# aouyang1/go-muse

Measured on NVIDIA B200. Metric: series-samples/sec (and % HBM roofline) for Batch.Run at 1/2/4/8 B200 vs host Go, higher is better.
Workload: dtype f64

## Files before the change

### go-muse_b200/csrc/muse_api.cu

```cuda
#include <cuda_runtime.h>

#include <algorithm>
#include <cmath>
#include <cstdarg>
#include <cstdio>
#include <cstdlib>
#include <cstring>
#include <atomic>
#include <mutex>
#include <thread>
#include <unordered_map>
#include <vector>

#include "../../include/muse_b200.h"
#include "muse_launch.h"
#include "muse_select.cuh"
#include "muse_synth.cuh"
#include "muse_xcorr.cuh"

using namespace muse;

static thread_local char g_err[512] = "";

static int fail(int code, const char *fmt, ...) {
    va_list ap;
    va_start(ap, fmt);
    vsnprintf(g_err, sizeof(g_err), fmt, ap);
    va_end(ap);
    return code;
}

static int cuda_fail(cudaError_t e, const char *call, const char *file, int line) {
    (void)cudaGetLastError();
    return fail(e == cudaErrorMemoryAllocation ? MUSE_ERR_OUT_OF_MEMORY : MUSE_ERR_CUDA, "%s failed: %s (%s:%d)", call,
                cudaGetErrorString(e), file, line);
}

#define CU(call)                                                                 \
    do {                                                                         \
        cudaError_t e_ = (call);                                                 \
        if (e_ != cudaSuccess) return cuda_fail(e_, #call, __FILE__, __LINE__); \
    } while (0)

extern "C" const char *muse_last_error(void) { return g_err; }
extern "C" const char *muse_version(void) { return "muse_b200 0.1 (sm_100a)"; }

#define MUSE_MAX_LABEL_KEYS 64
#define MUSE_SCRATCH_POOL 272
#define MUSE_MULTI_GROUP 256
#define MUSE_MULTI_SEPARATE 16
struct RunScratch {
    int64_t scratch_cap;
    double *d_score;
    int32_t *d_lag;
    int64_t *d_slot;
    unsigned long long *d_ckey, *d_skey;
    int32_t *d_cidx, *d_sidx;
    int32_t *d_clag, *d_slag;
    float *d_U;
    int32_t *d_list;
    float *d_L;
    signed char *d_W;
    int64_t d_L_cap;
    unsigned char *h_pin;
    size_t h_pin_bytes;
    unsigned long long *d_counters;
    SelectState *d_sel;
    int32_t *d_flag;
    unsigned *d_cut;
    int64_t table_cap;
    unsigned long long *d_gmax, *d_hkeys;
    int32_t *d_gidx;
    int64_t tab_n, d_ref_cap;
    int tab_screen;
    double *d_ref;
    cd *Xt, *twM, *twn;
    cf *twp_f;
    cf *twi_f;
    float2 *swtw;
    float4 *sw_f;
    float4 *sx_f;
    float *sb_f;
    float *d_mid;
    cudaEvent_t ev[4];
};

struct muse_ctx {
    int device;
    int sm_count;
    cudaStream_t stream;
    cudaStream_t own_stream;
    std::mutex mu;
    std::vector<RunScratch> pool;
    unsigned char *h_stage[3];
    cudaEvent_t stage_ev[3];
    double *d_roll;
    size_t d_roll_bytes;
    unsigned char *tc_a, *tc_b;
    size_t tc_a_bytes;
    float *tc_mid, *tc_amid;
    int64_t tc_mid_cap;
    void **tc_ptrs;
    unsigned *d_multi_next;
    unsigned char *d_mt, *h_mt;
    int64_t mt_top_n;
    cudaEvent_t mt_ev[5];
    int64_t multi_refined, multi_rescored;
    void *d_multi_q;
    double *d_multi_refs;
    int64_t d_multi_ld, d_multi_n;
};

struct muse_group {
    muse_ctx *ctx;
    int64_t N;
    int64_t ld;
    int64_t cap, size;
    double *slab;
    int nkeys;
    int32_t *labels;
    int32_t max_id[MUSE_MAX_LABEL_KEYS];
    int64_t global_offset;
    RowStat *row_stat;
    int64_t stats_cap, stats_upto;
};

struct muse_batch : RunScratch {
    muse_ctx *ctx;
    muse_group *g;
    int64_t N, n;
    int log2m;
    int screen_ok;
    float a_mid;
    cf x_mid;
    muse_timing timing;
    int timing_pending;
    int fused_run;
    int prescreened;
    int signed_run;
    int is_long;
    void *d_long;
    size_t d_long_bytes;
    long long long_pairs;
};

static inline cudaStream_t bstream(const muse_batch *b) { return b->ctx->stream; }

extern "C" int muse_ctx_create(int device, muse_ctx **out) {
    if (!out) return fail(MUSE_ERR_INVALID_ARG, "muse_ctx_create: out is NULL");
    int count = 0;
    cudaError_t e = cudaGetDeviceCount(&count);
    if (e != cudaSuccess || count == 0)
        return fail(MUSE_ERR_NO_DEVICE, "no CUDA device (%s); muse_b200 has no CPU fallback",
                    e != cudaSuccess ? cudaGetErrorString(e) : "device count is 0");
    if (device < 0 || device >= count) return fail(MUSE_ERR_INVALID_ARG, "device %d out of range [0,%d)", device, count);
    CU(cudaSetDevice(device));
    muse_ctx *c = new muse_ctx();
    c->device = device;
    CU(cudaDeviceGetAttribute(&c->sm_count, cudaDevAttrMultiProcessorCount, device));
    CU(cudaStreamCreateWithFlags(&c->own_stream, cudaStreamNonBlocking));
// ... 510 lines not shown
    int rc = roll_check(g, first, n_rows, samples, k, "muse_group_roll");
    if (rc != MUSE_OK || k == 0 || n_rows == 0) return rc;
    const size_t row_bytes = sizeof(double) * (size_t)k;
    if (row_bytes > MUSE_STAGE_BYTES) return fail(MUSE_ERR_UNSUPPORTED, "muse_group_roll: %lld new samples per row exceed the %zu-byte staging buffer",
                                                  (long long)k, MUSE_STAGE_BYTES);
    muse_ctx *c = g->ctx;
    CU(cudaSetDevice(c->device));
    cudaStream_t st = c->stream;
    const int64_t rows_per_chunk = stage_rows_per_chunk(k);
    const size_t want = row_bytes * (size_t)std::min<int64_t>(n_rows, rows_per_chunk);
    if (c->d_roll_bytes < want) {
        CU(cudaStreamSynchronize(st));
        cudaFree(c->d_roll);
        c->d_roll = nullptr;
        c->d_roll_bytes = 0;
        CU(cudaMalloc(&c->d_roll, want));
        c->d_roll_bytes = want;
    }
    auto queue = [&](int64_t r0, int64_t nr, const double *src) {
        cudaError_t e = cudaMemcpyAsync(c->d_roll, src, (size_t)nr * row_bytes, cudaMemcpyHostToDevice, st);
        if (e == cudaSuccess) e = launch_roll_rows(g->slab, g->ld, (int)g->N, first + r0, nr, c->d_roll, (int)k, g->row_stat, c->sm_count, st);
        return e;
    };
    cudaPointerAttributes attr;
    const bool pinned = cudaPointerGetAttributes(&attr, samples) == cudaSuccess &&
                        (attr.type == cudaMemoryTypeHost || attr.type == cudaMemoryTypeManaged);
    (void)cudaGetLastError();
    if (pinned) {
        for (int64_t r0 = 0; r0 < n_rows; r0 += rows_per_chunk)
            CU(queue(r0, std::min<int64_t>(rows_per_chunk, n_rows - r0), samples + (size_t)r0 * (size_t)k));
    } else {
        rc = stage_rows(c, samples, n_rows, k, queue);
        if (rc != MUSE_OK) return rc;
    }
    CU(cudaStreamSynchronize(st));
    return MUSE_OK;
}

static int64_t next_pow2(int64_t v) {
    int64_t n = 1;
    while (n < v) n <<= 1;
    return n;
}

static int screen_is_fused(int log2m) { return log2m >= 6 && log2m <= 13; }
static int screen_is_big(int log2m) { return log2m >= 11 && log2m <= 13; }

__global__ void screen_tables_kernel(const cd *__restrict__ Xt, int M, const float2 *__restrict__ swtw, float4 *__restrict__ sw,
                                     float4 *__restrict__ sx, float *__restrict__ sb, float *__restrict__ mid,
                                     const int32_t *__restrict__ std_zero) {
    const int k = blockIdx.x * blockDim.x + threadIdx.x;
    if (k > M / 2) return;
    if (k == 0) mid[0] = __int_as_float(*std_zero);
    const cd a = Xt[k], c = Xt[M - k];
    if (k == M / 2) {
        mid[1] = __double2float_ru(hypot(a.x, a.y) * 2.0);
        mid[2] = (float)a.x;
        mid[3] = (float)a.y;
        return;
    }
    const float wa = __double2float_ru(hypot(a.x, a.y) * (k == 0 ? 1.0 : 2.0));
    const float wc = __double2float_ru(hypot(c.x, c.y) * (k == 0 ? 1.0 : 2.0));
    const float2 w = swtw[k];
    sw[k] = make_float4(w.x, w.y, wa, wc);
    sx[k] = make_float4((float)a.x, (float)a.y, (float)c.x, (float)c.y);
    sb[k] = __double2float_ru(sqrt(2.0 * ((double)wa * (double)wa + (double)wc * (double)wc)) * (1.0 + 1e-15));
}

static int ensure_ref_tables(muse_batch *b, int64_t ld) {
    const int64_t n = b->n, M = n / 2;
    cudaStream_t st = bstream(b);
    if (b->d_ref_cap < ld) {
        cudaFree(b->d_ref);
        b->d_ref = nullptr;
        CU(cudaMalloc(&b->d_ref, sizeof(double) * (size_t)ld));
        b->d_ref_cap = ld;
    }
    if (!b->d_mid) CU(cudaMalloc(&b->d_mid, sizeof(float) * 4));
    const bool want_screen = screen_is_fused(b->log2m);
    if (b->tab_n == n && (b->tab_screen || !want_screen)) return MUSE_OK;
    if (b->is_long) {
        cudaFree(b->Xt); cudaFree(b->twM); cudaFree(b->twn); cudaFree(b->twp_f); cudaFree(b->twi_f); cudaFree(b->swtw); cudaFree(b->sw_f); cudaFree(b->sx_f); cudaFree(b->sb_f);
        b->Xt = b->twM = b->twn = nullptr;
        b->twp_f = b->twi_f = nullptr; b->swtw = nullptr; b->sw_f = b->sx_f = nullptr; b->sb_f = nullptr;
        b->tab_n = 0;
        b->tab_screen = 0;
        CU(cudaMalloc(&b->Xt, sizeof(cd) * (size_t)n));
        CU(cudaMalloc(&b->twM, sizeof(cd) * (size_t)n));
        CU(launch_long_twiddles(b->twM, b->log2m + 1, st));
        b->tab_n = n;
        return MUSE_OK;
    }
    cudaFree(b->Xt); cudaFree(b->twM); cudaFree(b->twn); cudaFree(b->twp_f); cudaFree(b->twi_f); cudaFree(b->swtw); cudaFree(b->sw_f); cudaFree(b->sx_f); cudaFree(b->sb_f);
    b->Xt = b->twM = b->twn = nullptr;
    b->twp_f = b->twi_f = nullptr; b->swtw = nullptr; b->sw_f = b->sx_f = nullptr; b->sb_f = nullptr;
    b->tab_n = 0;
    b->tab_screen = 0;
    const long double PI2 = 6.283185307179586476925286766559005768L;
    const int log2p = exact_log2p(b->log2m);
    std::vector<cd> twM((size_t)M + 16);
    fill_pass_twiddles(b->log2m, log2p, twM.data(), [&](long long num, long long den) {
        return cd{(double)cosl(-PI2 * num / den), (double)sinl(-PI2 * num / den)};
    });
    std::vector<cd> twn((size_t)(M / 2 + 1));
    for (int64_t k = 0; k <= M / 2; k++) twn[(size_t)k] = cd{(double)cosl(-PI2 * k / n), (double)sinl(-PI2 * k / n)};
    CU(cudaMalloc(&b->Xt, sizeof(cd) * (size_t)(M + 1)));
    CU(cudaMalloc(&b->twM, sizeof(cd) * twM.size()));
    CU(cudaMalloc(&b->twn, sizeof(cd) * (size_t)(M / 2 + 1)));
    CU(cudaMemcpyAsync(b->twM, twM.data(), sizeof(cd) * twM.size(), cudaMemcpyHostToDevice, st));
    CU(cudaMemcpyAsync(b->twn, twn.data(), sizeof(cd) * (size_t)(M / 2 + 1), cudaMemcpyHostToDevice, st));
    std::vector<cf> twp, twi;
    std::vector<float2> swtw;
    if (want_screen) {
        if (screen_is_big(b->log2m)) {
            twi.resize((size_t)10 * (M / 32) + 31 * (M / 1024) + 1024 + 31 * 32);
            fill_big_twiddles(b->log2m, twi.data(), [&](long long num, long long den) {
                return cf{(float)cosl(-PI2 * num / den), (float)sinl(-PI2 * num / den)};
            });
            CU(cudaMalloc(&b->twi_f, sizeof(cf) * twi.size()));
            CU(cudaMemcpyAsync(b->twi_f, twi.data(), sizeof(cf) * twi.size(), cudaMemcpyHostToDevice, st));
        }
        twp.resize((size_t)M + 64);
        fill_pass_twiddles(b->log2m, 5, twp.data(), [&](long long num, long long den) {
            return cf{(float)cosl(-PI2 * num / den), (float)sinl(-PI2 * num / den)};
        });
        swtw.resize((size_t)M / 2);
        for (int64_t k = 0; k < M / 2; k++) swtw[(size_t)k] = make_float2((float)cosl(-PI2 * k / n), (float)sinl(-PI2 * k / n));
        CU(cudaMalloc(&b->twp_f, sizeof(cf) * twp.size()));
        CU(cudaMalloc(&b->swtw, sizeof(float2) * swtw.size()));
        CU(cudaMalloc(&b->sw_f, sizeof(float4) * (size_t)(M / 2)));
        CU(cudaMalloc(&b->sx_f, sizeof(float4) * (size_t)(M / 2)));
        CU(cudaMalloc(&b->sb_f, sizeof(float) * (size_t)(M / 2)));
        CU(cudaMemcpyAsync(b->twp_f, twp.data(), sizeof(cf) * twp.size(), cudaMemcpyHostToDevice, st));
        CU(cudaMemcpyAsync(b->swtw, swtw.data(), sizeof(float2) * swtw.size(), cudaMemcpyHostToDevice, st));
    }
    CU(cudaStreamSynchronize(st));
    b->tab_n = n;
    b->tab_screen = want_screen ? 1 : 0;
    return MUSE_OK;
}

extern "C" void muse_batch_destroy(muse_batch *b);
static int ensure_long_work(muse_batch *b, int64_t count);
static LongParams long_params(const muse_batch *b, const double *slab, int64_t count, const int32_t *idx, int signed_scores);

#define CUB(call)                                                          \
    do {                                                                   \
        cudaError_t e_ = (call);                                           \
        if (e_ != cudaSuccess) {                                           \
            const int rc_ = cuda_fail(e_, #call, __FILE__, __LINE__);      \
            muse_batch_destroy(b);                                         \
            return rc_;                                                    \
        }                                                                  \
    } while (0)

static int batch_alloc(muse_ctx *ctx, muse_group *g, int64_t ref_len, muse_batch **out) {
    if (!ctx || !g || !out) return fail(MUSE_ERR_INVALID_ARG, "muse_batch_create: NULL argument");
    if (g->ctx != ctx) return fail(MUSE_ERR_INVALID_ARG, "group belongs to another context");
    if (ref_len != g->N)
        return fail(MUSE_ERR_LENGTH_MISMATCH, "comparison group series (length %lld) does not have the same length as the reference (%lld)",
                    (long long)g->N, (long long)ref_len);
    const int64_t n = next_pow2(ref_len);
    if (n > MUSE_MAX_FFT_LEN) return fail(MUSE_ERR_UNSUPPORTED, "FFT length %lld > %d", (long long)n, MUSE_MAX_FFT_LEN);
    CU(cudaSetDevice(ctx->device));
    muse_batch *b = new muse_batch();
    memset(b, 0, sizeof(*b));
    b->is_long = n > MUSE_MAX_FUSED_FFT_LEN;
    b->ctx = ctx;
    b->g = g;
    b->N = ref_len;
    b->n = n;
    const int64_t M = n / 2;
    int l = 0;
    while ((1LL << l) < M) l++;
    b->log2m = l;
    {
        std::lock_guard<std::mutex> lk(ctx->mu);
        if (!ctx->pool.empty()) {
            size_t best = 0;
            auto better = [&](const RunScratch &x, const RunScratch &y) {
                if ((x.tab_n == n) != (y.tab_n == n)) return x.tab_n == n;
                return x.scratch_cap > y.scratch_cap;
            };
            for (size_t i = 1; i < ctx->pool.size(); i++)
                if (better(ctx->pool[i], ctx->pool[best])) best = i;
            static_cast<RunScratch &>(*b) = ctx->pool[best];
            ctx->pool.erase(ctx->pool.begin() + (long)best);
        }
    }
    auto bail = [&](int code) {
        muse_batch_destroy(b);
        return code;
    };
    for (int i = 0; i < 4; i++)
        if (!b->ev[i] && cudaEventCreate(&b->ev[i]) != cudaSuccess) return bail(fail(MUSE_ERR_CUDA, "cudaEventCreate failed"));
    int rc = ensure_ref_tables(b, g->ld);
    if (rc) return bail(rc);
    cudaError_t e = cudaSuccess;
    if (!b->d_flag) e = cudaMalloc(&b->d_flag, sizeof(int32_t));
    if (e == cudaSuccess && !b->d_counters) e = cudaMalloc(&b->d_counters, sizeof(unsigned long long) * 4);
    if (e == cudaSuccess && !b->d_sel) e = cudaMalloc(&b->d_sel, sizeof(SelectState));
    if (e == cudaSuccess && !b->d_cut) e = cudaMalloc(&b->d_cut, sizeof(unsigned) * (4 + MUSE_CUT_WORDS));
    if (e == cudaSuccess && !b->h_pin) {
        b->h_pin_bytes = (size_t)4 << 20;
        e = cudaHostAlloc((void **)&b->h_pin, b->h_pin_bytes, cudaHostAllocDefault);
    }
    if (e != cudaSuccess) {
        (void)cudaGetLastError();
        return bail(fail(e == cudaErrorMemoryAllocation ? MUSE_ERR_OUT_OF_MEMORY : MUSE_ERR_CUDA, "muse_batch_create: %s", cudaGetErrorString(e)));
    }
    *out = b;
    return MUSE_OK;
}

static int batch_create_queue(muse_ctx *ctx, muse_group *g, const double *ref, int64_t ref_len, muse_batch **out,
                              const double *d_ref_row = nullptr) {
// ... 1819 lines not shown
```

### go-muse_b200/csrc/muse_screen.cuh

```cuda
#pragma once

#include <vector_functions.h>
#include <vector_types.h>

#include "muse_score.cuh"

namespace muse {

typedef cx<float> cf;

#ifndef MUSE_SCREEN_SLACK
#define MUSE_SCREEN_SLACK 1e-4f
#endif
#define MUSE_SCREEN_VAR_MIN 1e-20f
#define MUSE_SCREEN_VAR_MAX 1e28f
#define MUSE_SCREEN_OFFSET_MAX 1e8
#define MUSE_CUT_BINS 262144
#define MUSE_CUT_WORDS (64 + 64 * 64 + MUSE_CUT_BINS)

struct alignas(16) RowStat {
    double mean;
    float rstd;
    unsigned pad;
};

struct ScreenParams {
    const double *slab;
    int64_t ld;
    int64_t count;
    int N;
    const cf *twp;
    const float4 *sw;
    const float *sb;
    float a_mid;
    const float4 *sx;
    cf x_mid;
    float *out_L;
    const RowStat *row_stat;
    unsigned *cut_bits;
    unsigned *cut_hist;
    unsigned long long *n_refined;
    unsigned *next_claim;
    int top_n;
    int win_lo, win_len;
    float thr;
    int grouped;
    float *out_U;
    const cf *twi;
    const int64_t *slot_of;
    unsigned long long *group_L;
    signed char *out_W;
};

MUSE_HD bool window_row_hit(int off, int row_len, int win_lo, int win_len, int n) {
    const int d = (off - win_lo) & (n - 1);
    return d <= win_len || d > n - row_len;
}
MUSE_HD void window_pair(cx<float> r, int idx, int win_len, int nmask, bool hit, float &m_in, float &m_out) {
    const float a0 = fabsf(r.y), a1 = fabsf(r.x);
    if (hit) {
        const bool in0 = (idx & nmask) <= win_len;
        const bool in1 = ((idx + 1) & nmask) <= win_len;
        m_in = fmaxf(m_in, fmaxf(in0 ? a0 : 0.f, in1 ? a1 : 0.f));
        m_out = fmaxf(m_out, fmaxf(in0 ? 0.f : a0, in1 ? 0.f : a1));
    } else {
        m_out = fmaxf(m_out, fmaxf(a0, a1));
    }
}

#if defined(__CUDACC__)

template <int T>
__device__ __forceinline__ float group_sum_f(float x) {
#pragma unroll
    for (int off = T / 2; off > 0; off >>= 1) x += __shfl_xor_sync(0xffffffffu, x, off);
    return x;
}

__device__ __forceinline__ unsigned smem_u32(const void *p) { return (unsigned)__cvta_generic_to_shared(p); }

__device__ __forceinline__ void mbar_init(unsigned bar, unsigned count) {
    asm volatile("mbarrier.init.shared::cta.b64 [%0], %1;" ::"r"(bar), "r"(count) : "memory");
}
__device__ __forceinline__ void mbar_init_fence() { asm volatile("fence.mbarrier_init.release.cluster;" ::: "memory"); }
__device__ __forceinline__ void mbar_expect(unsigned bar, unsigned bytes) {
    asm volatile("mbarrier.arrive.expect_tx.shared::cta.b64 _, [%0], %1;" ::"r"(bar), "r"(bytes) : "memory");
}
__device__ __forceinline__ void bulk_copy(unsigned dst, const void *src, unsigned bytes, unsigned bar) {
    asm volatile("cp.async.bulk.shared::cluster.global.mbarrier::complete_tx::bytes [%0], [%1], %2, [%3];" ::"r"(dst), "l"(src),
                 "r"(bytes), "r"(bar)
                 : "memory");
}
__device__ __forceinline__ void bulk_load(unsigned dst, const void *src, unsigned bytes, unsigned bar) {
    mbar_expect(bar, bytes);
    bulk_copy(dst, src, bytes, bar);
}
__device__ __forceinline__ void mbar_wait(unsigned bar, unsigned parity) {
    unsigned done;
    do {
        asm volatile(
            "{\n"
            ".reg .pred p;\n"
            "mbarrier.try_wait.parity.shared::cta.b64 p, [%1], %2;\n"
            "selp.u32 %0, 1, 0, p;\n"
            "}\n"
            : "=r"(done)
            : "r"(bar), "r"(parity)
            : "memory");
    } while (!done);
}

__device__ __forceinline__ float sqrt_approx(float x) {
    float r;
    asm("sqrt.approx.ftz.f32 %0, %1;" : "=f"(r) : "f"(x));
    return r;
}

__device__ __forceinline__ unsigned ld_relaxed_u32(const unsigned *p) {
    unsigned r;
    asm volatile("ld.relaxed.gpu.global.u32 %0, [%1];" : "=r"(r) : "l"(p) : "memory");
    return r;
}

__device__ __forceinline__ void mbar_test(unsigned bar, unsigned parity) {
    asm volatile(
        "{\n"
        ".reg .pred p;\n"
        "mbarrier.test_wait.parity.shared::cta.b64 p, [%0], %1;\n"
        "}\n" ::"r"(bar),
        "r"(parity)
        : "memory");
}

__device__ __forceinline__ int cut_level(const unsigned *cnt, int t, unsigned &need) {
    const unsigned h = ld_relaxed_u32(&cnt[63 - 2 * t]), l = ld_relaxed_u32(&cnt[62 - 2 * t]);
    unsigned incl = h + l;
#pragma unroll
    for (int off = 1; off < 32; off <<= 1) {
        const unsigned o = __shfl_up_sync(0xffffffffu, incl, off);
        if (t >= off) incl += o;
    }
    const unsigned excl = incl - (h + l);
    const unsigned hit = __ballot_sync(0xffffffffu, incl >= need);
    if (!hit) return -1;
    const int leader = __ffs(hit) - 1;
    const bool upper = excl + h >= need;
    const int idx = upper ? 63 - 2 * t : 62 - 2 * t;
    const unsigned above = upper ? excl : excl + h;
    need -= __shfl_sync(0xffffffffu, above, leader);
    return __shfl_sync(0xffffffffu, idx, leader);
}

__device__ __forceinline__ void cut_count_and_raise(unsigned *const &cut_bits, unsigned *const &cut_hist, const int &top_n, float L, int t) {
    int bin = (int)(L * (float)MUSE_CUT_BINS);
    bin = bin < 0 ? 0 : (bin >= MUSE_CUT_BINS ? MUSE_CUT_BINS - 1 : bin);
    unsigned *coarse = cut_hist, *mid = coarse + 64, *fine = mid + 64 * 64;
    if (t == 0) {
        atomicAdd(&fine[bin], 1u);
        atomicAdd(&mid[bin >> 6], 1u);
        atomicAdd(&coarse[bin >> 12], 1u);
    }
    __syncwarp();
    unsigned need = (unsigned)top_n;
    const int c = cut_level(coarse, t, need);
    if (c < 0) return;
    const int m = cut_level(mid + c * 64, t, need);
    if (m < 0) return;
    const int f = cut_level(fine + (c * 64 + m) * 64, t, need);
    if (f < 0) return;
    if (t == 0) atomicMax(cut_bits, __float_as_uint((float)((c * 64 + m) * 64 + f) / (float)MUSE_CUT_BINS));
}

__device__ __forceinline__ float refine_decide(float U, float s_in, float s_out, float &L, int grouped) {
    if (!(s_in == s_in) || !(s_out == s_out)) return U;
    const float u32 = fminf(fmaxf(s_in, s_out) * 1.00001f, 1.f) + MUSE_SCREEN_SLACK;
    if (grouped) {
        L = fmaxf(fminf(fmaxf(s_in, s_out) * 0.99999f, 1.f) - MUSE_SCREEN_SLACK, 0.f);
        return fminf(U, u32);
    }
    if (s_out * 0.99999f - MUSE_SCREEN_SLACK > s_in * 1.00001f + MUSE_SCREEN_SLACK) return -1.f;
    if (s_in * 0.99999f - MUSE_SCREEN_SLACK > s_out * 1.00001f + MUSE_SCREEN_SLACK)
        L = fminf(s_in * 0.99999f, 1.f) - MUSE_SCREEN_SLACK;
    return fminf(U, u32);
}


template <int T>
MUSE_HD constexpr int screen_reg(int m) {
    return (m % (32 / T)) * T + Perm<T>::at(m / (32 / T));
}

template <int NZ, int T>
__device__ __forceinline__ void load_centred(cf (&v)[32], const cd *rowc, int t, double mu, bool last_in) {
#pragma unroll
    for (int r = 0; r < 32; r++) {
        if (r < NZ) {
            const cd x = (r == NZ - 1 && !last_in) ? cd{mu, mu} : rowc[t + r * T];
            v[r] = cf{(float)(x.x - mu), (float)(x.y - mu)};
        } else {
            v[r] = cf{0.f, 0.f};
        }
    }
}

template <int T>
__device__ __forceinline__ void screen_pass0(cf (&v)[32], cf *ex, const cf *const &tw, int t) {
    constexpr int LOG2M = 5 + (T >= 2) + (T >= 4) + (T >= 8) + (T >= 16) + (T >= 32);
    using G = Geo<LOG2M, 5>;
#pragma unroll
    for (int j = 0; j < 32; j++) {
        cf val = v[Perm<32>::at(j)];
        if (j > 0) val = cmul(val, tw[(j - 1) * T + t]);
        ex[G::pad(32 * t + j)] = val;
    }
    __syncwarp();
    fft_pass_load<LOG2M, 5, 1, float>(v, ex, t);
}

template <int T>
__device__ __forceinline__ void screen_pass1(cf *v) {
#pragma unroll
    for (int c = 0; c < 32 / T; c++) Dft<T, float>::run(v + c * T);
}

template <int T>
__device__ __forceinline__ cf mirror_of(const cf (&v)[32], int m, bool lane0, int partner) {
    const cf zp = v[screen_reg<T>(31 - m)];
    const cf zs = v[screen_reg<T>((32 - m) & 31)];
    cf src, zm;
    src.x = lane0 ? zs.x : zp.x;
    src.y = lane0 ? zs.y : zp.y;
    zm.x = __shfl_sync(0xffffffffu, src.x, partner, T);
    zm.y = __shfl_sync(0xffffffffu, src.y, partner, T);
    return zm;
}

__device__ __forceinline__ void split_sq(cf e, cf d, cf w, cf &qk, cf &qm) {
    const cf wo = cmul(cmul_negi(d), w);
    const cf y1 = cadd(e, wo);
    const cf y2 = csub(e, wo);
    qk = pmul(y1, y1);
    qm = pmul(y2, y2);
}

template <int T, bool PAIR>
__device__ __forceinline__ float screen_bound(const cf (&v)[32], const ScreenParams &prm, int t, bool lane0, int partner) {
    float acc = 0.f;
#pragma unroll
    for (int m = 0; m < 16; m++) {
        const cf zk = v[screen_reg<T>(m)];
        const cf zm = mirror_of<T>(v, m, lane0, partner);
        const cf zmc = cconj(zm);
        const cf e = cadd(zk, zmc);
        if constexpr (PAIR) {
            const cf d = csub(zk, zmc);
            const cf q = pfma(d, d, pmul(e, e));
            acc = fmaf(sqrt_approx(q.x + q.y), prm.sb[t + T * m], acc);
        } else {
            const float4 sv = prm.sw[t + T * m];
            cf qk, qm;
            split_sq(e, csub(zk, zmc), cf{sv.x, sv.y}, qk, qm);
            acc = fmaf(sqrt_approx(qk.x + qk.y), sv.z, fmaf(sqrt_approx(qm.x + qm.y), sv.w, acc));
        }
    }
    {
        const cf z = v[screen_reg<T>(16)];
        const cf q = pmul(z, z);
        acc = fmaf(sqrt_approx(q.x + q.y), lane0 ? 2.f * prm.a_mid : 0.f, acc);
    }
    return group_sum_f<T>(acc);
}

__device__ __forceinline__ cf split_twiddle(float4 s) { return cf{s.x, s.y}; }
__device__ __forceinline__ cf split_twiddle(cf s) { return s; }

template <int T, typename SW>
__device__ __forceinline__ void conj_mul_pairs(cf (&v)[32], const SW *const &sw, const float4 *const &sx, const cf &x_mid, int t, bool lane0,
                                               int partner) {
#pragma unroll
    for (int m = 0; m < 16; m++) {
        const cf zk = v[screen_reg<T>(m)];
        const cf zm = mirror_of<T>(v, m, lane0, partner);
        const cf w = split_twiddle(sw[t + T * m]);
        const float4 x = sx[t + T * m];
        cf ok, om;
        pointwise_pair(zk, zm, w, cf{x.x, x.y}, cf{x.z, x.w}, ok, om);
        cf rcv;
        rcv.x = __shfl_sync(0xffffffffu, om.x, partner, T);
        rcv.y = __shfl_sync(0xffffffffu, om.y, partner, T);
        v[screen_reg<T>(m)] = ok;
        cf &hi = v[screen_reg<T>(31 - m)];
        hi.x = lane0 ? hi.x : rcv.x;
        hi.y = lane0 ? hi.y : rcv.y;
        if (m > 0) {
            cf &own = v[screen_reg<T>(32 - m)];
            own.x = lane0 ? om.x : own.x;
// ... 47 lines not shown
    return r;
}

struct RowSums {
    double s1 = 0.0, s2 = 0.0;
    __device__ __forceinline__ void add(double v, double pivot) {
        const double x = v - pivot;
        s1 += x;
        s2 = fma(x, x, s2);
    }
    __device__ __forceinline__ RowStat warp_stat(double pivot, int N) {
#pragma unroll
        for (int off = 16; off > 0; off >>= 1) {
            s1 += __shfl_xor_sync(0xffffffffu, s1, off);
            s2 += __shfl_xor_sync(0xffffffffu, s2, off);
        }
        return make_row_stat(pivot, s1, s2, N);
    }
};
#endif

static __global__ void row_stats_kernel(double *__restrict__ slab, int64_t ld, int N, int64_t first, int64_t count,
                                 RowStat *__restrict__ stat) {
    const int lane = threadIdx.x & 31;
    const int64_t warp0 = ((int64_t)blockIdx.x * blockDim.x + threadIdx.x) >> 5;
    const int64_t nwarp = ((int64_t)gridDim.x * blockDim.x) >> 5;
    for (int64_t i = warp0; i < count; i += nwarp) {
        const double *row = slab + (first + i) * ld;
        const double pivot = row[0];
        RowSums rs;
        for (int k = lane; k < N; k += 32) rs.add(row[k], pivot);
        const RowStat r = rs.warp_stat(pivot, N);
        if (lane == 0) {
            stat[first + i] = r;
            if (N & 1) slab[(first + i) * ld + N] = r.mean;
        }
    }
}

struct ScreenWarpCfg {
    using G = Geo<10, 5>;
    static constexpr int MAX_WARPS = 12;
    static constexpr int NREF = 2;
    static constexpr int CLAIM = 2;
    static constexpr size_t SMEM_BUDGET = 227 * 1024;
    static constexpr size_t EX_BYTES = ((size_t)(G::MP + 1) * sizeof(cf) + 127) / 128 * 128;
    static size_t row_bytes(int N) { const size_t r = ((size_t)N * 8 + 127) / 128 * 128; return r > EX_BYTES ? r : EX_BYTES; }
    static size_t warp_bytes(int N) { return row_bytes(N); }
    static int warps(int N) {
        const size_t w = (SMEM_BUDGET - NREF * EX_BYTES) / warp_bytes(N);
        return (int)(w > MAX_WARPS ? MAX_WARPS : w);
    }
    static size_t smem_bytes(int N) { return (size_t)warps(N) * warp_bytes(N) + NREF * EX_BYTES; }
    static int nz(int N) { return ((N + 1) / 2 + 31) / 32; }
};

__device__ __forceinline__ int ex_acquire(unsigned *locks, int t, int hint) {
    int slot = hint & (ScreenWarpCfg::NREF - 1);
    while (true) {
        unsigned old = 1u;
        if (t == 0) old = atomicCAS(&locks[slot], 0u, 1u);
        if (__shfl_sync(0xffffffffu, old, 0) == 0u) break;
        slot = (slot + 1) & (ScreenWarpCfg::NREF - 1);
    }
    return slot;
}
__device__ __forceinline__ void ex_release(unsigned *locks, int t, int slot) {
    __syncwarp();
    if (t == 0) {
        __threadfence_block();
        atomicExch(&locks[slot], 0u);
    }
}

template <int NZ>
__global__ void __launch_bounds__(ScreenWarpCfg::MAX_WARPS * 32, 1)
score_screen_warp_kernel(const ScreenParams prm, const unsigned warp_bytes, const unsigned row_bytes) {
    using C = ScreenWarpCfg;
    constexpr int P = 32;
    extern __shared__ __align__(128) unsigned char smem_raw[];
    __shared__ __align__(8) unsigned long long bars[C::MAX_WARPS];
    __shared__ unsigned ex_locks[C::NREF];
    __shared__ int next_of[C::MAX_WARPS];

    const int w = threadIdx.x >> 5;
    const int t = threadIdx.x & 31;
    const int count = (int)prm.count;
    const int grid_warps = (int)(gridDim.x * (blockDim.x >> 5));
    const int pos0 = ((int)(blockIdx.x * (blockDim.x >> 5)) + w) * C::CLAIM;
    unsigned char *buf = smem_raw + (size_t)w * warp_bytes;
    const cd *rowc = reinterpret_cast<const cd *>(buf);
    cf *sm = reinterpret_cast<cf *>(buf);
    unsigned char *refbase = smem_raw + (size_t)(blockDim.x >> 5) * warp_bytes;
    const int N = prm.N;
    const int Nh = (N + 1) >> 1;
    const unsigned bar = smem_u32(&bars[w]);
    const int partner = (P - t) & (P - 1);
    const bool lane0 = (t == 0);
    const bool last_in = t + (NZ - 1) * 32 < Nh;

    if (threadIdx.x < C::NREF) ex_locks[threadIdx.x] = 0u;
    if (t == 0) {
        mbar_init(bar, 1);
        mbar_init_fence();
        if (pos0 < count) bulk_load(smem_u32(buf), prm.slab + (int64_t)pos0 * prm.ld, (unsigned)(N + (N & 1)) * 8u, bar);
    }
    __syncthreads();

    unsigned pp = (unsigned)pos0;
    while ((int)(pp & 0x7fffffffu) < count) {
        const int pos = (int)(pp & 0x7fffffffu);
        const unsigned phase = pp >> 31;
        const bool claim_ends = (pos & (C::CLAIM - 1)) == C::CLAIM - 1;
        unsigned cut_raw = 0u, claim = 0u;
        if (t == 0) {
            cut_raw = ld_relaxed_u32(prm.cut_bits);
            if (claim_ends) claim = atomicInc(prm.next_claim, (unsigned)count);
        }
        const RowStat rs = prm.row_stat[pos];
        const double mu = rs.mean;
        mbar_wait(bar, phase);

        cf v[P];
        load_centred<NZ, 32>(v, rowc, t, mu, last_in);
        __syncwarp();

        Dft32Lead<NZ, float>::run(v);
        screen_pass0<32>(v, sm, prm.twp, t);
        __syncwarp();
        if (t == 0) {
            const int next = claim_ends ? (grid_warps + (int)claim) * C::CLAIM : pos + 1;
            next_of[w] = next;
            if (next < count) {
                asm volatile("" ::"r"(__float_as_uint(v[P - 1].y)) : "memory");
                asm volatile("fence.proxy.async.shared::cta;" ::: "memory");
                bulk_load(smem_u32(buf), prm.slab + (int64_t)next * prm.ld, (unsigned)(N + (N & 1)) * 8u, bar);
            }
        }
        screen_pass1<32>(v);
        const float acc = screen_bound<32, true>(v, prm, t, lane0, partner);

        float U = acc * rs.rstd * 1.00001f + MUSE_SCREEN_SLACK;
        if (!(U == U)) U = 2.f;
        float L = -1.f;
        const int bsrc = (__float_as_uint(acc) == 0x7fc12345u) ? 1 : 0;
        const float cut_now = __uint_as_float(__shfl_sync(0xffffffffu, cut_raw, bsrc));
        if (U >= cut_now && U < 1.5f) {
#pragma unroll
            for (int j = 0; j < P / 2; j++) {
                const cf zk = v[Perm<P>::at(j)];
                const cf zm = mirror_of<32>(v, j, lane0, partner);
                const float4 s = prm.sw[t + 32 * j];
                const float4 x = prm.sx[t + 32 * j];
                cf ok, om;
                pointwise_pair(zk, zm, cf{s.x, s.y}, cf{x.x, x.y}, cf{x.z, x.w}, ok, om);
                cf rcv;
                rcv.x = __shfl_sync(0xffffffffu, om.x, partner);
                rcv.y = __shfl_sync(0xffffffffu, om.y, partner);
                v[Perm<P>::at(j)] = ok;
                cf &hi = v[Perm<P>::at(P - 1 - j)];
                hi.x = lane0 ? hi.x : rcv.x;
                hi.y = lane0 ? hi.y : rcv.y;
                if (j > 0) {
                    cf &own = v[Perm<P>::at(P - j)];
                    own.x = lane0 ? om.x : own.x;
                    own.y = lane0 ? om.y : own.y;
                }
            }
            {
                cf &mid = v[Perm<P>::at(P / 2)];
                cf ok, om;
                pointwise_pair(mid, mid, cf{0.f, -1.f}, prm.x_mid, prm.x_mid, ok, om);
                mid.x = lane0 ? ok.x : mid.x;
                mid.y = lane0 ? ok.y : mid.y;
            }
            cf u[P];
#pragma unroll
            for (int j = 0; j < P; j++) u[j] = v[Perm<P>::at(j)];
            Dft<P, float>::run(u);
            {
                const int slot = ex_acquire(ex_locks, t, w);
                screen_pass0<32>(u, reinterpret_cast<cf *>(refbase + (size_t)slot * C::EX_BYTES), prm.twp, t);
                ex_release(ex_locks, t, slot);
            }
            screen_pass1<32>(u);
            float m_in, m_out;
            window_maxima<32>(u, t, prm.win_lo, prm.win_len, m_in, m_out);
            const float rstd = rs.rstd;
            const float s_in = m_in * rstd, s_out = m_out * rstd;
            U = refine_decide(U, s_in, s_out, L, prm.grouped);
            if (t == 0) atomicAdd(prm.n_refined, 1ull);
            if (L >= prm.thr && L >= cut_now) cut_count_and_raise(prm.cut_bits, prm.cut_hist, prm.top_n, L, t);
        }
        if (t == 0) {
            prm.out_U[pos] = U;
            if (prm.out_L) prm.out_L[pos] = L;
        }
        __syncwarp();
        pp = (unsigned)next_of[w] | (~pp & 0x80000000u);
    }
}

#endif

}
```

### go-muse_b200/csrc/muse_screen_big.cuh

```cuda
#pragma once

#include "muse_screen.cuh"

namespace muse {

template <int LOG2M>
struct ScreenBigCfg {
    static_assert(LOG2M >= 11 && LOG2M <= 13, "big kernel: n = 4096, 8192, 16384");
    static constexpr int M = 1 << LOG2M;
    static constexpr int P = 32;
    static constexpr int T = M / P;
    static constexpr int NWARP = T / 32;
    static constexpr int LR = LOG2M - 10;
    static constexpr int R = 1 << LR;
    static constexpr int NB = P / R;
    static constexpr int NPAIR = NB / 2;
    static constexpr int TP = T + (T >> 5);
    static constexpr int JP = 1024 + 32;
    static constexpr int TR = T + (T >> LR);
    static constexpr int SM_ELEMS = M + (M >> LR) + 2;
    static constexpr size_t EX_BYTES = ((size_t)SM_ELEMS * 8 + 127) / 128 * 128;
#ifndef MUSE_BIG_SMEM_TW
#define MUSE_BIG_SMEM_TW 1
#endif
// ... 200 lines not shown
            }
        } else {
#pragma unroll
            for (int j = 0; j < R; j++) {
                cf &a = lo[Perm<R>::at(j)], &b = hi[Perm<R>::at(R - 1 - j)];
                cf ok, om;
                if (j < R / 2) {
                    const float4 s = big_load_f4(sw + u + 1024 * j), x = big_load_f4(sx + u + 1024 * j);
                    pointwise_pair(a, b, cf{s.x, s.y}, cf{x.x, x.y}, cf{x.z, x.w}, ok, om);
                    a = ok;
                    b = om;
                } else {
                    const int kk = M - u - 1024 * j;
                    const float4 s = big_load_f4(sw + kk), x = big_load_f4(sx + kk);
                    pointwise_pair(b, a, cf{s.x, s.y}, cf{x.x, x.y}, cf{x.z, x.w}, ok, om);
                    b = ok;
                    a = om;
                }
            }
        }
    }
}

template <int LOG2M>
MUSE_HD void big_inv_pass0(cf *v, cf *sm, int t, const cf *twi) {
    using C = ScreenBigCfg<LOG2M>;
    constexpr int R = C::R;
#pragma unroll
    for (int c2 = 0; c2 < C::NPAIR; c2++) {
        const int u = t + C::T * c2;
#pragma unroll
        for (int h = 0; h < 2; h++) {
            const int b = h == 0 ? u : big_b_hi(u);
            cf *x = v + (2 * c2 + h) * R;
            cf w[R];
#pragma unroll
            for (int j = 0; j < R; j++) w[j] = x[Perm<R>::at(j)];
            Dft<R, float>::run(w);
            cf *dst = sm + (R + 1) * b;
            dst[0] = w[Perm<R>::at(0)];
            cf pw[R];
            pw[1] = twi[C::TWI0_OFF + b];
#pragma unroll
            for (int j = 2; j < R; j++) pw[j] = cmul(pw[j / 2], pw[j - j / 2]);
#pragma unroll
            for (int j = 1; j < R; j++) dst[j] = cmul(w[Perm<R>::at(j)], pw[j]);
        }
    }
}
template <int LOG2M>
MUSE_HD void big_inv_pass1_load(cf *v, const cf *sm, int t) {
    using C = ScreenBigCfg<LOG2M>;
    const int ptr = t + (t >> C::LR);
#pragma unroll
    for (int j = 0; j < 32; j++) v[j] = sm[ptr + C::TR * j];
}
template <int LOG2M>
MUSE_HD void big_inv_pass1(cf *v, cf *sm, int t, const cf *twi) {
    using C = ScreenBigCfg<LOG2M>;
    constexpr int R = C::R;
    Dft<32, float>::run(v);
    const int p = t >> C::LR, q = t & (R - 1);
    cf *dst = sm + q + 33 * R * p;
    const cf *tw = twi + C::TWI1_OFF + p;
    dst[0] = v[Perm<32>::at(0)];
#pragma unroll
    for (int j = 1; j < 32; j++) dst[R * j + ((R * j) >> 5)] = cmul(v[Perm<32>::at(j)], tw[(j - 1) * 32]);
}
template <int LOG2M>
MUSE_HD void big_window_max(const cf *v, int t, int win_lo, int win_len, float &m_in, float &m_out) {
    using C = ScreenBigCfg<LOG2M>;
    m_in = 0.f;
    m_out = 0.f;
    const int base = 2 * t - win_lo;
#pragma unroll
    for (int j = 0; j < 32; j++) {
        const int off = 2 * C::T * j;
        window_pair(v[Perm<32>::at(j)], base + off, win_len, 2 * C::M - 1, window_row_hit(off, 2 * C::T, win_lo, win_len, 2 * C::M), m_in,
                    m_out);
    }
}

#if defined(__CUDACC__)

__device__ __forceinline__ void big_l2_prefetch(const void *p, unsigned bytes) {
    asm volatile("cp.async.bulk.prefetch.L2.global [%0], %1;" ::"l"(p), "r"(bytes) : "memory");
}

#ifndef MUSE_BIG_LOAD_BATCH
#define MUSE_BIG_LOAD_BATCH 16
#endif

template <int LOG2M, int MINB, int NZ = 0>
__global__ void __launch_bounds__(ScreenBigCfg<LOG2M>::T, MINB)
score_screen_big_kernel(const ScreenParams prm) {
    using C = ScreenBigCfg<LOG2M>;
    constexpr int P = 32, T = C::T, NW = C::NWARP, LB = MUSE_BIG_LOAD_BATCH;
    extern __shared__ __align__(128) unsigned char smem_raw[];
    __shared__ float2 red_f[2][NW];
    __shared__ unsigned bc_word[2];
    cf *sm = reinterpret_cast<cf *>(smem_raw);
#if MUSE_BIG_SMEM_TW
    cf *s_tw = reinterpret_cast<cf *>(smem_raw + C::EX_BYTES);
    for (int i = threadIdx.x; i < C::TW_SMEM; i += C::T) s_tw[i] = prm.twi[i];
    float *s_sb = reinterpret_cast<float *>(s_tw + C::TW_SMEM);
    if (C::SB_SMEM)
        for (int i = threadIdx.x; i < C::M / 2; i += C::T) s_sb[i] = prm.sb[i];
    __syncthreads();
    const cf *twf = s_tw;
    const cf *twinv = MUSE_BIG_SMEM_TW == 3 ? s_tw : prm.twi;
    const float *sbp = C::SB_SMEM ? s_sb : prm.sb;
#else
    const cf *twf = prm.twi;
    const cf *twinv = prm.twi;
    const float *sbp = prm.sb;
#endif

    const int t = threadIdx.x;
    const int N = prm.N;
    const int Nh = (N + 1) >> 1;
    const int count = (int)prm.count;
    const unsigned row_bytes = (unsigned)(N + (N & 1)) * 8u;
    const int chunk = (count + (int)gridDim.x - 1) / (int)gridDim.x;
    const int pos_lo = (int)blockIdx.x * chunk;
    const int pos_hi = min(pos_lo + chunk, count);
    if (t == 0 && pos_lo < pos_hi) big_l2_prefetch(prm.slab + (int64_t)pos_lo * prm.ld, row_bytes);

    for (int pos = pos_lo; pos < pos_hi; pos++) {
        const double *rowp = prm.slab + (int64_t)pos * prm.ld;
        unsigned cut_raw = 0u, lg_raw = 0u;
        unsigned long long *gslot = nullptr;
        if (t == 0) {
            if (pos + 1 < pos_hi) big_l2_prefetch(rowp + prm.ld, row_bytes);
            cut_raw = ld_relaxed_u32(prm.cut_bits);
            if (prm.group_L) {
                gslot = prm.group_L + prm.slot_of[pos];
                lg_raw = ld_relaxed_u32(reinterpret_cast<const unsigned *>(gslot));
            }
        }
        const RowStat rs = prm.row_stat[pos];
        const double mu = rs.mean;

        cf v[P];
#pragma unroll
        for (int b0 = 0; b0 < P; b0 += LB) {
            cd x[LB];
#pragma unroll
            for (int q = 0; q < LB; q++) {
                const int j = t + (b0 + q) * T;
if constexpr (NZ > 0) {
                    if (b0 + q < NZ - 1) x[q] = load_pair_stream(rowp + 2 * j);
                    else if (b0 + q == NZ - 1) x[q] = j < Nh ? load_pair_stream(rowp + 2 * j) : cd{mu, mu};
                    else x[q] = cd{mu, mu};
                } else {
                    x[q] = (b0 + q < P / 2 || j < Nh) ? load_pair_stream(rowp + 2 * j) : cd{mu, mu};
                }
            }
#pragma unroll
            for (int q = 0; q < LB; q++) {
                if (NZ > 0 && b0 + q >= NZ) v[b0 + q] = cf{0.f, 0.f};
                else v[b0 + q] = cf{(float)(x[q].x - mu), (float)(x[q].y - mu)};
            }
        }

        big_fwd_pass0<LOG2M, NZ == 0 ? 32 : NZ>(v, sm, t, twf);
        __syncthreads();
        big_load_stride_t<LOG2M>(v, sm, t);
        __syncthreads();
        big_fwd_pass1<LOG2M>(v, sm, t, twf);
        __syncthreads();
        big_fwd_last<LOG2M>(v, sm, t);

#if defined(MUSE_BIG_BINS)
        float acc = big_split_bound<LOG2M, false>(v, t, prm.sw, prm.a_mid, sbp);
#else
        float acc = big_split_bound<LOG2M, true>(v, t, prm.sw, prm.a_mid, sbp);
#endif
#pragma unroll
        for (int off = 16; off > 0; off >>= 1) acc += __shfl_xor_sync(0xffffffffu, acc, off);
        if ((t & 31) == 0) red_f[0][t >> 5].x = acc;
        if (t == 0) {
            bc_word[0] = cut_raw;
            bc_word[1] = lg_raw;
        }
        __syncthreads();
        acc = red_f[0][0].x;
#pragma unroll
        for (int w = 1; w < NW; w++) acc += red_f[0][w].x;
        const float cut_now = __uint_as_float(bc_word[0]);
        const float lg_now = __uint_as_float(bc_word[1]);
        float U = acc * rs.rstd * 1.00001f + MUSE_SCREEN_SLACK;
        if (!(U == U)) U = 2.f;
        float L = -1.f;
        signed char W = 0;
        if (U >= cut_now && U >= lg_now && U < 1.5f) {
            big_pointwise<LOG2M>(v, t, prm.sw, prm.sx, prm.x_mid);
            big_inv_pass0<LOG2M>(v, sm, t, twinv);
            __syncthreads();
            big_inv_pass1_load<LOG2M>(v, sm, t);
            __syncthreads();
            big_inv_pass1<LOG2M>(v, sm, t, twinv);
            __syncthreads();
            big_load_stride_t<LOG2M>(v, sm, t);
            Dft<32, float>::run(v);
            float m_in, m_out;
            big_window_max<LOG2M>(v, t, prm.win_lo, prm.win_len, m_in, m_out);
#pragma unroll
            for (int off = 16; off > 0; off >>= 1) {
                m_in = fmaxf(m_in, __shfl_xor_sync(0xffffffffu, m_in, off));
                m_out = fmaxf(m_out, __shfl_xor_sync(0xffffffffu, m_out, off));
            }
            if ((t & 31) == 0) red_f[1][t >> 5] = make_float2(m_in, m_out);
            __syncthreads();
            float2 mx = red_f[1][0];
#pragma unroll
            for (int w = 1; w < NW; w++) {
// ... 29 lines not shown
```

### go-muse_b200/csrc/muse_screen_multi.cuh

```cuda
#pragma once

#include "muse_screen.cuh"

namespace muse {

struct MultiQuery {
    const float4 *sw;
    const float4 *sx;
    cf x_mid;
    float a_mid;
    int pad;
    unsigned *cut;
    float *out_U;
};

#if defined(__CUDACC__)

struct RefineMultiCfg {
    using G = Geo<10, 5>;
#ifndef MUSE_REFINE_WARPS
#define MUSE_REFINE_WARPS 8
#endif
    static constexpr int MAX_WARPS = MUSE_REFINE_WARPS;
    static constexpr int QMAX = 256;
    static constexpr int QI = QMAX / 32;
    static constexpr size_t SMEM_BUDGET = 227 * 1024;
    static constexpr size_t STASH_BYTES = (size_t)G::M * sizeof(cf);
    static constexpr size_t EX_BYTES = ScreenWarpCfg::EX_BYTES;
    static size_t warp_bytes(int N) {
        const size_t row = ((size_t)N * 8 + 127) / 128 * 128, own = STASH_BYTES + EX_BYTES;
        return row > own ? row : own;
    }
    static constexpr size_t TW_BYTES = 31 * 32 * sizeof(cf) + 64, SW_BYTES = (size_t)(G::M / 2) * sizeof(cf);
    static size_t table_bytes() { return (size_t)QMAX * 2 * sizeof(void *) + TW_BYTES + SW_BYTES; }
    static int warps(int N) {
        const size_t w = (SMEM_BUDGET - table_bytes()) / warp_bytes(N);
        return (int)(w > MAX_WARPS ? MAX_WARPS : w);
    }
    static size_t smem_bytes(int N) { return (size_t)warps(N) * warp_bytes(N) + table_bytes(); }
};

template <int NZ>
__global__ void __launch_bounds__(RefineMultiCfg::MAX_WARPS * 32, 1)
refine_multi_kernel(const ScreenParams prm, const MultiQuery *__restrict__ queries, const int nq, const unsigned warp_bytes,
                    unsigned *__restrict__ next_series) {
    using C = RefineMultiCfg;
    constexpr int P = 32, M = C::G::M, QI = C::QI;
    extern __shared__ __align__(128) unsigned char smem_raw[];
    __shared__ __align__(8) unsigned long long bars[C::MAX_WARPS];

    const int w = threadIdx.x >> 5;
    const int t = threadIdx.x & 31;
    const int nwarps = (int)(blockDim.x >> 5);
    const int count = (int)prm.count;
    const int pos0 = (int)(blockIdx.x * nwarps) + w;
    unsigned char *buf = smem_raw + (size_t)w * warp_bytes;
    const cd *rowc = reinterpret_cast<const cd *>(buf);
    cf *stash = reinterpret_cast<cf *>(buf);
    cf *ex = reinterpret_cast<cf *>(buf + C::STASH_BYTES);
    unsigned **s_cut = reinterpret_cast<unsigned **>(smem_raw + (size_t)nwarps * warp_bytes);
    float **s_out = reinterpret_cast<float **>(s_cut + C::QMAX);
    cf *s_tw = reinterpret_cast<cf *>(s_out + C::QMAX);
    cf *s_sw = reinterpret_cast<cf *>(reinterpret_cast<unsigned char *>(s_tw) + C::TW_BYTES);
    const int N = prm.N;
    const int Nh = (N + 1) >> 1;
    const unsigned bar = smem_u32(&bars[w]);
    const int partner = (P - t) & (P - 1);
    const bool lane0 = (t == 0);
    const bool last_in = t + (NZ - 1) * 32 < Nh;
    const int nqi = (nq + 31) >> 5;

    if (t == 0) {
        mbar_init(bar, 1);
        mbar_init_fence();
        if (pos0 < count) bulk_load(smem_u32(buf), prm.slab + (int64_t)pos0 * prm.ld, (unsigned)(N + (N & 1)) * 8u, bar);
    }
    for (int q = threadIdx.x; q < C::QMAX; q += blockDim.x) {
        s_cut[q] = q < nq ? queries[q].cut : nullptr;
        s_out[q] = q < nq ? queries[q].out_U : nullptr;
    }
    for (int i = threadIdx.x; i < 31 * 32; i += blockDim.x) s_tw[i] = prm.twp[i];
    for (int i = threadIdx.x; i < M / 2; i += blockDim.x) {
        const float4 s = prm.sw[i];
        s_sw[i] = cf{s.x, s.y};
    }
    __syncthreads();

    unsigned phase = 0;
    int next = 0;
    for (int pos = pos0; pos < count; pos = next, phase ^= 1u) {
        float U[QI];
        unsigned cutr[QI];
#pragma unroll
        for (int i = 0; i < QI; i++) {
            U[i] = -1.f;
            cutr[i] = 0x7f800000u;
            if (i < nqi && t + 32 * i < nq) {
                U[i] = s_out[t + 32 * i][pos];
                cutr[i] = ld_relaxed_u32(s_cut[t + 32 * i]);
            }
        }
        const RowStat rs = prm.row_stat[pos];
        const double mu = rs.mean;
        mbar_wait(bar, phase);

        cf v[P];
        load_centred<NZ, 32>(v, rowc, t, mu, last_in);
        __syncwarp();
        if (t == 0) next = (int)atomicAdd(next_series, 1u);
        next = __shfl_sync(0xffffffffu, next, 0);

        Dft32Lead<NZ, float>::run(v);
        screen_pass0<32>(v, ex, s_tw, t);
        screen_pass1<32>(v);
#pragma unroll
        for (int j = 0; j < P; j++) stash[32 * j + t] = v[Perm<P>::at(j)];

        unsigned todo[QI];
#pragma unroll
        for (int i = 0; i < QI; i++) todo[i] = __ballot_sync(0xffffffffu, U[i] >= __uint_as_float(cutr[i]) && U[i] < 1.5f);
        unsigned changed = 0u;
#pragma unroll 1
        while (true) {
            int gi = -1;
            unsigned gm = 0u;
#pragma unroll
            for (int i = QI - 1; i >= 0; i--)
                if (todo[i]) {
                    gi = i;
                    gm = todo[i];
                }
            if (gi < 0) break;
            const int ql = __ffs(gm) - 1;
            float Usel = 0.f;
            unsigned csel = 0u;
#pragma unroll
            for (int i = 0; i < QI; i++) {
                if (i == gi) {
                    todo[i] = gm & (gm - 1);
                    Usel = U[i];
                    csel = cutr[i];
                }
            }
            {
                float Uq = __shfl_sync(0xffffffffu, Usel, ql);
                const float cut_now = __uint_as_float(__shfl_sync(0xffffffffu, csel, ql));
                const MultiQuery mq = queries[32 * gi + ql];
                cf z[P];
#pragma unroll
                for (int j = 0; j < P; j++) z[Perm<P>::at(j)] = stash[32 * j + t];
                conj_mul_pairs<32>(z, s_sw, mq.sx, mq.x_mid, t, lane0, partner);
                cf u[P];
#pragma unroll
                for (int j = 0; j < P; j++) u[j] = z[Perm<P>::at(j)];
                Dft<P, float>::run(u);
                __syncwarp();
                screen_pass0<32>(u, ex, s_tw, t);
                screen_pass1<32>(u);
                float m_in, m_out;
                window_maxima<32>(u, t, prm.win_lo, prm.win_len, m_in, m_out);
                float L = -1.f;
                Uq = refine_decide(Uq, m_in * rs.rstd, m_out * rs.rstd, L, 0);
                if (t == 0) atomicAdd(reinterpret_cast<unsigned long long *>(mq.cut + 2), 1ull);
                if (L >= prm.thr && L >= cut_now) cut_count_and_raise(mq.cut, mq.cut + 4, prm.top_n, L, t);
// ... 23 lines not shown
```

Baseline: 664.1 billion.

## Pack screen pass twiddles as float4 pairs and prefetch next claimed rows into L2

Repacks the float screen FFT pass-0 twiddle table so each thread loads two twiddles per float4 (odd/even j pairs). This halves the number of twiddle loads in screen_pass0. The single-query screen kernel now claims its next row block at the start of a claim instead of the end, and uses that early claim to issue a bulk L2 prefetch of the upcoming rows. The cost is an extra shared-memory slot per warp and an earlier atomic. The L2 prefetch helper is also shared with the big-screen kernel.

```diff
diff --git a/go-muse_b200/csrc/muse_api.cu b/go-muse_b200/csrc/muse_api.cu
--- a/go-muse_b200/csrc/muse_api.cu
+++ b/go-muse_b200/csrc/muse_api.cu
@@ -75,7 +75,7 @@
     int tab_screen;
     double *d_ref;
     cd *Xt, *twM, *twn;
-    cf *twp_f;
+    float4 *twp_f;
     cf *twi_f;
     float2 *swtw;
     float4 *sw_f;
@@ -752,7 +752,7 @@
     if (b->is_long) {
         cudaFree(b->Xt); cudaFree(b->twM); cudaFree(b->twn); cudaFree(b->twp_f); cudaFree(b->twi_f); cudaFree(b->swtw); cudaFree(b->sw_f); cudaFree(b->sx_f); cudaFree(b->sb_f);
         b->Xt = b->twM = b->twn = nullptr;
-        b->twp_f = b->twi_f = nullptr; b->swtw = nullptr; b->sw_f = b->sx_f = nullptr; b->sb_f = nullptr;
+        b->twp_f = nullptr; b->twi_f = nullptr; b->swtw = nullptr; b->sw_f = b->sx_f = nullptr; b->sb_f = nullptr;
         b->tab_n = 0;
         b->tab_screen = 0;
         CU(cudaMalloc(&b->Xt, sizeof(cd) * (size_t)n));
@@ -763,7 +763,7 @@
     }
     cudaFree(b->Xt); cudaFree(b->twM); cudaFree(b->twn); cudaFree(b->twp_f); cudaFree(b->twi_f); cudaFree(b->swtw); cudaFree(b->sw_f); cudaFree(b->sx_f); cudaFree(b->sb_f);
     b->Xt = b->twM = b->twn = nullptr;
-    b->twp_f = b->twi_f = nullptr; b->swtw = nullptr; b->sw_f = b->sx_f = nullptr; b->sb_f = nullptr;
+    b->twp_f = nullptr; b->twi_f = nullptr; b->swtw = nullptr; b->sw_f = b->sx_f = nullptr; b->sb_f = nullptr;
     b->tab_n = 0;
     b->tab_screen = 0;
     const long double PI2 = 6.283185307179586476925286766559005768L;
@@ -779,7 +779,8 @@
     CU(cudaMalloc(&b->twn, sizeof(cd) * (size_t)(M / 2 + 1)));
     CU(cudaMemcpyAsync(b->twM, twM.data(), sizeof(cd) * twM.size(), cudaMemcpyHostToDevice, st));
     CU(cudaMemcpyAsync(b->twn, twn.data(), sizeof(cd) * (size_t)(M / 2 + 1), cudaMemcpyHostToDevice, st));
-    std::vector<cf> twp, twi;
+    std::vector<float4> twp;
+    std::vector<cf> twi;
     std::vector<float2> swtw;
     if (want_screen) {
         if (screen_is_big(b->log2m)) {
@@ -790,18 +791,22 @@
             CU(cudaMalloc(&b->twi_f, sizeof(cf) * twi.size()));
             CU(cudaMemcpyAsync(b->twi_f, twi.data(), sizeof(cf) * twi.size(), cudaMemcpyHostToDevice, st));
         }
-        twp.resize((size_t)M + 64);
-        fill_pass_twiddles(b->log2m, 5, twp.data(), [&](long long num, long long den) {
-            return cf{(float)cosl(-PI2 * num / den), (float)sinl(-PI2 * num / den)};
-        });
+        const int64_t T = M / 32;
+        twp.resize((size_t)(16 * T));
+        for (int64_t i = 0; i < 16; i++)
+            for (int64_t t = 0; t < T; t++) {
+                const int64_t k1 = (2 * i + 1) * t, k2 = (2 * i + 2) * t;
+                twp[(size_t)(i * T + t)] = make_float4((float)cosl(-PI2 * k1 / M), (float)sinl(-PI2 * k1 / M), (float)cosl(-PI2 * k2 / M),
+                                                       (float)sinl(-PI2 * k2 / M));
+            }
         swtw.resize((size_t)M / 2);
         for (int64_t k = 0; k < M / 2; k++) swtw[(size_t)k] = make_float2((float)cosl(-PI2 * k / n), (float)sinl(-PI2 * k / n));
-        CU(cudaMalloc(&b->twp_f, sizeof(cf) * twp.size()));
+        CU(cudaMalloc(&b->twp_f, sizeof(float4) * twp.size()));
         CU(cudaMalloc(&b->swtw, sizeof(float2) * swtw.size()));
         CU(cudaMalloc(&b->sw_f, sizeof(float4) * (size_t)(M / 2)));
         CU(cudaMalloc(&b->sx_f, sizeof(float4) * (size_t)(M / 2)));
         CU(cudaMalloc(&b->sb_f, sizeof(float) * (size_t)(M / 2)));
-        CU(cudaMemcpyAsync(b->twp_f, twp.data(), sizeof(cf) * twp.size(), cudaMemcpyHostToDevice, st));
+        CU(cudaMemcpyAsync(b->twp_f, twp.data(), sizeof(float4) * twp.size(), cudaMemcpyHostToDevice, st));
         CU(cudaMemcpyAsync(b->swtw, swtw.data(), sizeof(float2) * swtw.size(), cudaMemcpyHostToDevice, st));
     }
     CU(cudaStreamSynchronize(st));
diff --git a/go-muse_b200/csrc/muse_screen.cuh b/go-muse_b200/csrc/muse_screen.cuh
--- a/go-muse_b200/csrc/muse_screen.cuh
+++ b/go-muse_b200/csrc/muse_screen.cuh
@@ -29,7 +29,7 @@
     int64_t ld;
     int64_t count;
     int N;
-    const cf *twp;
+    const float4 *twp;
     const float4 *sw;
     const float *sb;
     float a_mid;
@@ -91,6 +91,9 @@
                  "r"(bytes), "r"(bar)
                  : "memory");
 }
+__device__ __forceinline__ void l2_prefetch(const void *p, unsigned bytes) {
+    asm volatile("cp.async.bulk.prefetch.L2.global [%0], %1;" ::"l"(p), "r"(bytes) : "memory");
+}
 __device__ __forceinline__ void bulk_load(unsigned dst, const void *src, unsigned bytes, unsigned bar) {
     mbar_expect(bar, bytes);
     bulk_copy(dst, src, bytes, bar);
@@ -204,14 +207,16 @@
 }
 
 template <int T>
-__device__ __forceinline__ void screen_pass0(cf (&v)[32], cf *ex, const cf *const &tw, int t) {
+__device__ __forceinline__ void screen_pass0(cf (&v)[32], cf *ex, const float4 *const &tw, int t) {
     constexpr int LOG2M = 5 + (T >= 2) + (T >= 4) + (T >= 8) + (T >= 16) + (T >= 32);
     using G = Geo<LOG2M, 5>;
-#pragma unroll
-    for (int j = 0; j < 32; j++) {
-        cf val = v[Perm<32>::at(j)];
-        if (j > 0) val = cmul(val, tw[(j - 1) * T + t]);
-        ex[G::pad(32 * t + j)] = val;
+    const float4 *twt = tw + t;
+    ex[G::pad(32 * t)] = v[0];
+#pragma unroll
+    for (int j = 1; j < 32; j += 2) {
+        const float4 w = twt[(j >> 1) * T];
+        ex[G::pad(32 * t + j)] = cmul(v[Perm<32>::at(j)], cf{w.x, w.y});
+        if (j < 31) ex[G::pad(32 * t + j + 1)] = cmul(v[Perm<32>::at(j + 1)], cf{w.z, w.w});
     }
     __syncwarp();
     fft_pass_load<LOG2M, 5, 1, float>(v, ex, t);
@@ -425,6 +430,7 @@
     __shared__ __align__(8) unsigned long long bars[C::MAX_WARPS];
     __shared__ unsigned ex_locks[C::NREF];
     __shared__ int next_of[C::MAX_WARPS];
+    __shared__ int claim_of[C::MAX_WARPS];
 
     const int w = threadIdx.x >> 5;
     const int t = threadIdx.x & 31;
@@ -454,11 +460,20 @@
     while ((int)(pp & 0x7fffffffu) < count) {
         const int pos = (int)(pp & 0x7fffffffu);
         const unsigned phase = pp >> 31;
+        const bool claim_starts = (pos & (C::CLAIM - 1)) == 0;
         const bool claim_ends = (pos & (C::CLAIM - 1)) == C::CLAIM - 1;
         unsigned cut_raw = 0u, claim = 0u;
         if (t == 0) {
             cut_raw = ld_relaxed_u32(prm.cut_bits);
-            if (claim_ends) claim = atomicInc(prm.next_claim, (unsigned)count);
+            if (claim_starts) {
+                claim = atomicInc(prm.next_claim, (unsigned)count);
+            } else if (claim_ends) {
+                const int nc = claim_of[w];
+                if (nc < count) {
+                    const int rows = count - nc < C::CLAIM ? count - nc : C::CLAIM;
+                    l2_prefetch(prm.slab + (int64_t)nc * prm.ld, (unsigned)((int64_t)(rows - 1) * prm.ld + N + (N & 1)) * 8u);
+                }
+            }
         }
         const RowStat rs = prm.row_stat[pos];
         const double mu = rs.mean;
@@ -472,7 +487,8 @@
         screen_pass0<32>(v, sm, prm.twp, t);
         __syncwarp();
         if (t == 0) {
-            const int next = claim_ends ? (grid_warps + (int)claim) * C::CLAIM : pos + 1;
+            if (claim_starts) claim_of[w] = (grid_warps + (int)claim) * C::CLAIM;
+            const int next = claim_ends ? claim_of[w] : pos + 1;
             next_of[w] = next;
             if (next < count) {
                 asm volatile("" ::"r"(__float_as_uint(v[P - 1].y)) : "memory");
diff --git a/go-muse_b200/csrc/muse_screen_big.cuh b/go-muse_b200/csrc/muse_screen_big.cuh
--- a/go-muse_b200/csrc/muse_screen_big.cuh
+++ b/go-muse_b200/csrc/muse_screen_big.cuh
@@ -306,10 +306,6 @@
 }
 
 #if defined(__CUDACC__)
-
-__device__ __forceinline__ void big_l2_prefetch(const void *p, unsigned bytes) {
-    asm volatile("cp.async.bulk.prefetch.L2.global [%0], %1;" ::"l"(p), "r"(bytes) : "memory");
-}
 
 #ifndef MUSE_BIG_LOAD_BATCH
 #define MUSE_BIG_LOAD_BATCH 16
@@ -348,14 +344,14 @@
     const int chunk = (count + (int)gridDim.x - 1) / (int)gridDim.x;
     const int pos_lo = (int)blockIdx.x * chunk;
     const int pos_hi = min(pos_lo + chunk, count);
-    if (t == 0 && pos_lo < pos_hi) big_l2_prefetch(prm.slab + (int64_t)pos_lo * prm.ld, row_bytes);
+    if (t == 0 && pos_lo < pos_hi) l2_prefetch(prm.slab + (int64_t)pos_lo * prm.ld, row_bytes);
 
     for (int pos = pos_lo; pos < pos_hi; pos++) {
         const double *rowp = prm.slab + (int64_t)pos * prm.ld;
         unsigned cut_raw = 0u, lg_raw = 0u;
         unsigned long long *gslot = nullptr;
         if (t == 0) {
-            if (pos + 1 < pos_hi) big_l2_prefetch(rowp + prm.ld, row_bytes);
+            if (pos + 1 < pos_hi) l2_prefetch(rowp + prm.ld, row_bytes);
             cut_raw = ld_relaxed_u32(prm.cut_bits);
             if (prm.group_L) {
                 gslot = prm.group_L + prm.slot_of[pos];
diff --git a/go-muse_b200/csrc/muse_screen_multi.cuh b/go-muse_b200/csrc/muse_screen_multi.cuh
--- a/go-muse_b200/csrc/muse_screen_multi.cuh
+++ b/go-muse_b200/csrc/muse_screen_multi.cuh
@@ -31,7 +31,7 @@
         const size_t row = ((size_t)N * 8 + 127) / 128 * 128, own = STASH_BYTES + EX_BYTES;
         return row > own ? row : own;
     }
-    static constexpr size_t TW_BYTES = 31 * 32 * sizeof(cf) + 64, SW_BYTES = (size_t)(G::M / 2) * sizeof(cf);
+    static constexpr size_t TW_BYTES = 16 * 32 * sizeof(float4), SW_BYTES = (size_t)(G::M / 2) * sizeof(cf);
     static size_t table_bytes() { return (size_t)QMAX * 2 * sizeof(void *) + TW_BYTES + SW_BYTES; }
     static int warps(int N) {
         const size_t w = (SMEM_BUDGET - table_bytes()) / warp_bytes(N);
@@ -60,7 +60,7 @@
     cf *ex = reinterpret_cast<cf *>(buf + C::STASH_BYTES);
     unsigned **s_cut = reinterpret_cast<unsigned **>(smem_raw + (size_t)nwarps * warp_bytes);
     float **s_out = reinterpret_cast<float **>(s_cut + C::QMAX);
-    cf *s_tw = reinterpret_cast<cf *>(s_out + C::QMAX);
+    float4 *s_tw = reinterpret_cast<float4 *>(s_out + C::QMAX);
     cf *s_sw = reinterpret_cast<cf *>(reinterpret_cast<unsigned char *>(s_tw) + C::TW_BYTES);
     const int N = prm.N;
     const int Nh = (N + 1) >> 1;
@@ -79,7 +79,7 @@
         s_cut[q] = q < nq ? queries[q].cut : nullptr;
         s_out[q] = q < nq ? queries[q].out_U : nullptr;
     }
-    for (int i = threadIdx.x; i < 31 * 32; i += blockDim.x) s_tw[i] = prm.twp[i];
+    for (int i = threadIdx.x; i < 16 * 32; i += blockDim.x) s_tw[i] = prm.twp[i];
     for (int i = threadIdx.x; i < M / 2; i += blockDim.x) {
         const float4 s = prm.sw[i];
         s_sw[i] = cf{s.x, s.y};
```

Measured after the change: 627.4 billion, median of 6. 5.5% lower.
